# limix/CellRegMap

Hardware: AMD Instinct MI355X
Metric: variant-tests/sec (interaction test) (higher is better)
Workload: dtype f64

## Files before the change

cellregmap_amd/_lib.py:

```python
import ctypes
import os

import numpy as np

_HERE = os.path.dirname(os.path.abspath(__file__))
LIB_PATH = os.path.join(_HERE, "libcrm_hip.so")

c_double_p = ctypes.POINTER(ctypes.c_double)
c_int_p = ctypes.POINTER(ctypes.c_int)
c_long_p = ctypes.POINTER(ctypes.c_long)
vp = ctypes.c_void_p

SIGNATURES = {
    "crm_last_error": (ctypes.c_char_p, []),
    "crm_version": (ctypes.c_char_p, []),
    "crm_ctx_create": (ctypes.c_int, [ctypes.c_int, ctypes.POINTER(vp)]),
    "crm_ctx_destroy": (None, [vp]),
    "crm_ctx_synchronize": (ctypes.c_int, [vp]),
    "crm_ctx_trim": (ctypes.c_int, [vp]),
    "crm_background_create_qs": (ctypes.c_int, [vp, ctypes.c_long, ctypes.c_int, vp, vp, vp, vp,
                                                ctypes.POINTER(vp)]),
    "crm_background_create": (ctypes.c_int, [vp, ctypes.c_long, vp, ctypes.c_int, vp, ctypes.c_long,
                                             ctypes.c_int, vp, ctypes.c_double, ctypes.POINTER(vp)]),
    "crm_background_create_hadamard": (ctypes.c_int, [vp, ctypes.c_long, vp, ctypes.c_int, vp, ctypes.c_int, vp,
# ... 50 lines not shown
    "crm_set_progress_callback": (ctypes.c_int, [vp, vp, vp]),
    "crm_set_fast_rotation": (ctypes.c_int, [vp, ctypes.c_int]),
    "crm_kernel_timer_reset": (ctypes.c_int, [vp]),
    "crm_kernel_timer_read": (ctypes.c_int, [vp, c_double_p, c_long_p, c_double_p, c_double_p]),
    "crm_kernel_timer_stop": (ctypes.c_int, [vp]),
    "crm_test_set_form": (ctypes.c_int, [ctypes.c_char_p, ctypes.c_int, ctypes.c_int]),
    "crm_test_set_contraction": (ctypes.c_int, [vp, ctypes.c_int, ctypes.c_int]),
    "crm_test_set_shared_h": (ctypes.c_int, [vp, ctypes.c_int]),
    "crm_test_tail_launches": (ctypes.c_long, [vp]),
    "crm_test_spectrum_tail_launches": (ctypes.c_long, [vp]),
    "crm_test_dense_repeats": (ctypes.c_long, [vp]),
    "crm_test_donor_pair_blocks": (ctypes.c_long, [vp]),
    "crm_test_unrelated_donor_blocks": (ctypes.c_int, [vp, ctypes.POINTER(ctypes.c_long)]),
    "crm_test_gram_dma_launches": (ctypes.c_int, [vp, ctypes.POINTER(ctypes.c_long)]),
    "crm_test_fused_blocks": (ctypes.c_int, [vp, ctypes.POINTER(ctypes.c_long)]),
    "crm_test_rho0_position_blocks": (ctypes.c_int, [vp, ctypes.POINTER(ctypes.c_long)]),
    "crm_test_rotation_tail_launches": (ctypes.c_int, [vp, ctypes.POINTER(ctypes.c_long)]),
    "crm_test_tests_without_pair": (ctypes.c_long, [vp]),
    "crm_test_set_contraction_sync": (ctypes.c_int, [vp, ctypes.c_int]),
    "crm_test_sync_fallbacks": (ctypes.c_long, [vp]),
    "crm_test_overruns": (ctypes.c_long, []),
    "crm_test_live_device_bytes": (ctypes.c_long, []),
    "crm_test_set_kinship_route": (ctypes.c_int, [vp, ctypes.c_int]),
    "crm_test_check_context": (ctypes.c_int, [vp]),
    "crm_test_overrun_selftest": (ctypes.c_int, [vp]),
    "crm_test_null_fit_probe": (ctypes.c_int, [vp, ctypes.c_int, ctypes.c_double]),
    "crm_test_null_fit_probe_read": (ctypes.c_int, [vp, vp, ctypes.c_long]),
    "crm_test_contract": (ctypes.c_int, [vp, ctypes.c_long, ctypes.c_int, ctypes.c_int, vp, vp, vp,
                                         ctypes.c_int]),
    "crm_test_contract_kr": (ctypes.c_int, [vp, ctypes.c_long, ctypes.c_int, ctypes.c_int, ctypes.c_int,
# ... 52 lines not shown
```

cellregmap_amd/csrc/api_core.hip:

```cpp
#include <dlfcn.h>

#include <algorithm>
#include <atomic>
#include <cstdarg>
#include <mutex>

#include <map>

#include "crm_internal.h"
#include "eigh.h"

namespace crm {

static thread_local std::string g_error;

void set_error(const char* fmt, ...) {
    char buf[1024];
    va_list ap;
    va_start(ap, fmt);
    vsnprintf(buf, sizeof buf, fmt, ap);
    va_end(ap);
    g_error = buf;
}

// ... 258 lines not shown
    if (!c) return CRM_ERR_ARG;
    c->fast_T = on != 0;
    return CRM_OK;
    });
}

extern "C++" {
namespace crm {
namespace {
struct FormSlot { const char* name; int value; bool set; };
FormSlot g_forms[] = {{"gram_staged", 0, false}, {"kr_no_tail", 0, false}, {"nullfit_per_wave", 0, false}, {"kin_fold", 0, false},
                      {"eigh_one_stage", 0, false}, {"nullfit_exact", 0, false}, {"donor_pairs", 0, false},
                      {"pairs_without_kinship_term", 0, false}, {"flat_kappa_milli", 0, false}, {"chase_abort", 0, false}, {"nullfit_one_per_wave", 0, false},
                      {"kin_diag", 0, false}, {"donor_pairs_rotate", 0, false}, {"rho0_positions", 0, false},
                      {"rotation_tails", 0, false}, {"woodbury_ytY", 0, false},
                      {"wb_block_order", 0, false}, {"block_fused", 0, false}};
std::mutex g_forms_mu;
}
int form(const char* name, int otherwise) {
    std::lock_guard<std::mutex> lock(g_forms_mu);
    for (const FormSlot& f : g_forms)
        if (strcmp(f.name, name) == 0) return f.set ? f.value : otherwise;
    return otherwise;
}
}
}

int crm_test_set_form(const char* name, int value, int reset) {
    return crm::guarded("crm_test_set_form", [&]() -> int {
    if (!name) return CRM_ERR_ARG;
    std::lock_guard<std::mutex> lock(crm::g_forms_mu);
// ... 23 lines not shown
    return CRM_OK;
    });
}
int crm_test_unrelated_donor_blocks(const crm_ctx* ctx, long* blocks) {
    return crm::guarded("crm_test_unrelated_donor_blocks", [&]() -> int {
    if (!ctx || !blocks) return CRM_ERR_ARG;
    *blocks = ctx->unrelated_donor_blocks;
    return CRM_OK;
    });
}

int crm_test_fused_blocks(const crm_ctx* ctx, long* blocks) {
    return crm::guarded("crm_test_fused_blocks", [&]() -> int {
    if (!ctx || !blocks) return CRM_ERR_ARG;
    *blocks = ctx->fused_blocks;
    return CRM_OK;
    });
}

int crm_test_rho0_position_blocks(const crm_ctx* ctx, long* blocks) {
    return crm::guarded("crm_test_rho0_position_blocks", [&]() -> int {
    if (!ctx || !blocks) return CRM_ERR_ARG;
    *blocks = ctx->rho0_position_blocks;
    return CRM_OK;
    });
}
int crm_test_rotation_tail_launches(const crm_ctx* ctx, long* launches) {
    return crm::guarded("crm_test_rotation_tail_launches", [&]() -> int {
    if (!ctx || !launches) return CRM_ERR_ARG;
    *launches = ctx->rotation_tail_launches;
// ... 323 lines not shown
```

cellregmap_amd/csrc/assemble.hip:

```cpp
#include <type_traits>

#include "nullfit.h"

namespace crm {

namespace {

constexpr int CH = 64;
constexpr int SLD = 66;

typedef double v4d __attribute__((ext_vector_type(4)));

template <int NTL, int NG = 1>
__global__ __launch_bounds__(256) void gram_ext_kernel(AssembleArgs a, double* __restrict__ Gext, int KT) {
    constexpr int ROWS = 16 * NTL, NTILES = NTL * (NTL + 1) / 2, NLOC = (NTILES + NG - 1) / NG, MAXT = (NLOC + 3) / 4,
                  RPT = ROWS / 4;
    extern __shared__ double Ss[];
    __shared__ int tile_ij[NTILES];
    __shared__ const double* tail_ptr[ROWS];
    const int b = blockIdx.x;
    const NullFitOut fit = a.fit[b];
    const AssembleRho R = a.rho[fit.rho_index];
    const int r = R.r;
    const double ratio = fit.v0 / fit.v1;
// ... 809 lines not shown
            return CRM_ERR_INTERNAL;
        }
        Gext = a.wb_Gw;
    }
    const int P = a.c + 1;
    const size_t fin_small = sizeof(double) * ((size_t)P * P + 3 * P + a.k0);
    size_t fin_lds = fin_small + sizeof(double) * 2 * (size_t)a.k0 * P;
    const bool rows_global = fin_lds > 150 * 1024;
    if (rows_global) fin_lds = fin_small;
    if (a.k0 > CRM_MAX_K0 || a.c > CRM_MAX_COV_XWIDE || KT > CRM_MAX_GRAM_ROWS || (rows_global && !fin_rows)) {
        set_error("assemble: k0=%d, c=%d outside the supported range (k0 <= %d, c <= %d, k0 + c + 2 <= %d)", a.k0, a.c,
                  CRM_MAX_K0, CRM_MAX_COV_XWIDE, CRM_MAX_GRAM_ROWS);
        return CRM_ERR_UNSUPPORTED;
    }
    const int ts = (KT + 15) / 16;
    bool dma = ts <= 9 && a.ldA % 2 == 0 && (reinterpret_cast<uintptr_t>(a.A) & 15) == 0 && !form("gram_staged", 0);
    for (int i = 0; dma && i < CRM_MAX_RHO; i++) {
        const AssembleRho& R = a.rho[i];
        if (R.r <= 0 && !R.ty) continue;
        dma = R.ldW % 2 == 0 && R.ldT % 2 == 0 && ((reinterpret_cast<uintptr_t>(R.ty) | reinterpret_cast<uintptr_t>(R.tW) |
                                                    reinterpret_cast<uintptr_t>(R.T)) & 15) == 0;
    }
    if (a.wb_k1 > 0) dma = dma && a.wb_ldR % 2 == 0 && (reinterpret_cast<uintptr_t>(a.wb_R) & 15) == 0;
#define CRM_GRAM_DMA(KERNEL, LDS_DOUBLES, NTL)                                                                \
    do {                                                                                                      \
        const size_t lds = sizeof(double) * LDS_DOUBLES(NTL);                                                 \
        if (lds > 60 * 1024)                                                                                  \
            CRM_HIP(hipFuncSetAttribute(reinterpret_cast<const void*>(&KERNEL<NTL>),                          \
                                        hipFuncAttributeMaxDynamicSharedMemorySize, (int)lds));               \
        hipLaunchKernelGGL(KERNEL<NTL>, dim3(variants), dim3(256), lds, st, a, Gext, KT);                     \
    } while (0)
#define CRM_GRAM_DMA_WIDE(NTL) CRM_GRAM_DMA(gram_ext_dma_wide_kernel, gram_dma_wide_lds_doubles, NTL)
    if (dma) {
        if (ts <= 2) CRM_GRAM_DMA(gram_ext_dma_kernel, gram_dma_lds_doubles, 2);
        else if (ts <= 4) CRM_GRAM_DMA(gram_ext_dma_kernel, gram_dma_lds_doubles, 4);
        else if (ts == 5) CRM_GRAM_DMA_WIDE(5);
        else if (ts == 6) CRM_GRAM_DMA_WIDE(6);
        else if (ts == 7) CRM_GRAM_DMA_WIDE(7);
        else if (ts == 8) CRM_GRAM_DMA_WIDE(8);
        else CRM_GRAM_DMA_WIDE(9);
    }
#undef CRM_GRAM_DMA_WIDE
#undef CRM_GRAM_DMA
#define CRM_GRAM(NTL)                                                                                         \
    do {                                                                                                      \
        const size_t lds = sizeof(double) * 16 * NTL * SLD;                                                   \
        if (lds > 60 * 1024)                                                                                  \
            CRM_HIP(hipFuncSetAttribute(reinterpret_cast<const void*>(&gram_ext_kernel<NTL>),                 \
                                        hipFuncAttributeMaxDynamicSharedMemorySize, (int)lds));               \
        hipLaunchKernelGGL(gram_ext_kernel<NTL>, dim3(variants), dim3(256), lds, st, a, Gext, KT);            \
    } while (0)
#define CRM_GRAM_GROUPS(NTL, NG)                                                                              \
    do {                                                                                                      \
        const size_t lds = sizeof(double) * 16 * NTL * SLD;                                                   \
        CRM_HIP(hipFuncSetAttribute(reinterpret_cast<const void*>(&gram_ext_kernel<NTL, NG>),                 \
                                    hipFuncAttributeMaxDynamicSharedMemorySize, (int)lds));                   \
        hipLaunchKernelGGL((gram_ext_kernel<NTL, NG>), dim3(variants, NG), dim3(256), lds, st, a, Gext, KT);  \
    } while (0)
    if (dma) {
    } else if (ts <= 2) CRM_GRAM(2);
    else if (ts <= 4) CRM_GRAM(4);
    else if (ts <= 6) CRM_GRAM(6);
    else if (ts <= 7) CRM_GRAM(7);
    else if (ts <= 9) CRM_GRAM(9);
    else if (ts <= 12) CRM_GRAM_GROUPS(12, 2);
    else if (ts <= 15) CRM_GRAM_GROUPS(15, 4);
    else CRM_GRAM_GROUPS(18, 4);
#undef CRM_GRAM
#undef CRM_GRAM_GROUPS
    CRM_HIP(hipGetLastError());
    if (dma && dma_launches) ++*dma_launches;
    const bool yty = a.wb_k1 > 0 && form("woodbury_ytY", 1) != 0;
    if (a.wb_k1 > 0) {
        const size_t lds = yty ? sizeof(double) * a.wb_k1 * (size_t)((KT0 + a.wb_k1) | 1) : woodbury_lds_bytes(KT0, a.wb_k1);
        const void* fn = yty ? reinterpret_cast<const void*>(&woodbury_yty_kernel) : reinterpret_cast<const void*>(&woodbury_kernel);
        if (lds > 60 * 1024) CRM_HIP(hipFuncSetAttribute(fn, hipFuncAttributeMaxDynamicSharedMemorySize, (int)lds));
        if (yty) hipLaunchKernelGGL(woodbury_yty_kernel, dim3(variants), dim3(256), lds, st, a, a.wb_Gw, KT0, Gfin);
        else hipLaunchKernelGGL(woodbury_kernel, dim3(variants), dim3(256), lds, st, a, a.wb_Gw, KT0, Gfin);
        CRM_HIP(hipGetLastError());
    }
    if (fin_lds > 60 * 1024)
        CRM_HIP(hipFuncSetAttribute(reinterpret_cast<const void*>(&finalize_kernel),
                                    hipFuncAttributeMaxDynamicSharedMemorySize, (int)fin_lds));
    hipLaunchKernelGGL(finalize_kernel, dim3(variants), dim3(128), fin_lds, st, a, Gfin, KT0, rows_global ? fin_rows : nullptr,
                       yty ? 1 : 0);
    CRM_HIP(hipGetLastError());
// ... 5 lines not shown
```

cellregmap_amd/csrc/crm_internal.h:

```cpp
#pragma once
#include <map>
#include <mutex>
#include <thread>
#include <type_traits>
#include <utility>

#include "crm_common.h"

namespace crm {

constexpr int CRM_DEFAULT_BLOCK = 1024;
constexpr int CRM_MAX_AUTO_BLOCK = 4096;
constexpr int CRM_MAX_RHO = 16;
constexpr int CRM_MAX_COV = 8;
constexpr int CRM_MAX_COV_WIDE = 62;
constexpr int CRM_MAX_COV_XWIDE = 128;
constexpr int CRM_MAX_K0 = 256;
constexpr int CRM_MAX_GRAM_ROWS = 288;
constexpr int DT_SUMS_LD = 136;
constexpr int BLOCK_SLACK_MAX = 4096;

struct DevBuf {
    void* ptr = nullptr;
    size_t bytes = 0;
// ... 57 lines not shown
    bool probe_on = false;
    int probe_mode = 0;
    double probe_x = 0.0;
    std::vector<double> probe_out;
    bool nullfit_exact = false;
    crm::GemmTune tune;
    crm::DevBuf sync_counters;
    unsigned* sync_timeouts_host = nullptr;
    long sync_fallbacks = 0;
    long dense_repeats = 0;
    long tail_launches = 0;
    long spectrum_tail_launches = 0;
    long donor_pair_blocks = 0;
    long rotation_tail_launches = 0;
    long rho0_position_blocks = 0;
    long fused_blocks = 0;
    long unrelated_donor_blocks = 0;
    long gram_dma_launches = 0;
    long tests_without_pair = 0;
    struct ReplayBlock {
        long col0 = 0;
        int nb = 0;
        bool collapsed = false;
        std::vector<char> fit;
        crm::DevBuf T;
    };
    int replay_mode = 0;
    size_t replay_cursor = 0;
    std::vector<ReplayBlock*> replay_blocks;
    void replay_clear() {
// ... 46 lines not shown
```

cellregmap_amd/csrc/nullfit.h:

```cpp
#pragma once
#include "crm_internal.h"

namespace crm {

struct NullFitRho {
    const double* T;
    const double* ty;
    const double* tW;
    const double* S0;
    long ldT, ldW;
    int r;
    int pad_;
};

struct NullFitTrial {
    double lml, delta, scale;
    int use_g, nfev;
    double margin;
    double noise;
    double curv;
};

struct NullFitOut {
    int rho_index;
// ... 153 lines not shown
    const double* Z1; long ldZ1;
    const double* Z2; long ldZ2;
    const double* Z3; long ldZ3;
    const double* WW; const double* Wy; double yy;
    const double* gg; const double* gy; const double* gW; long ld_gW;
    const double* coef; long ld_coef;
    double* Q;
    double* F;
    int wb_k1;
    const double* wb_R; long wb_ldR;
    const double* wb_E1X; long wb_ldE1X;
    const double* wb_E1yW; long wb_ldE1yW;
    const double* wb_E1g; long wb_ldE1g;
    const double* wb_EE;
    double* wb_Gw;
};

int launch_assemble(hipStream_t st, const AssembleArgs& a, int variants, double* Gext, double* fin_rows = nullptr,
                    long* dma_launches = nullptr);
size_t assemble_rows_scratch_doubles(int variants, int k0, int c);
size_t woodbury_lds_bytes(int KT, int k1);

int launch_eig_davies(hipStream_t st, const double* F, const double* Q, int count, int k,
                      double* lambda, double* pvalue, int* ifault, double* liu, bool do_eig, double* scratch = nullptr,
                      int* trace = nullptr);
size_t eig_scratch_doubles(int count, int k);

int launch_tail_pvalue(hipStream_t st, const double* Q, const double* lambda, int count, int k, double* pvalue,
                       double* logp, int* status);

}
```

cellregmap_amd/csrc/scan_pairs.hip:

```cpp
#include "scan_pass.h"

namespace crm {

SubRange ScanPass::sub_range(const Block& B, int b0) const {
    SubRange R;
    R.b0 = b0;
    R.nb = B.nb - b0;
    R.done = B.done + b0;
    if (ng > 1) {
        long pairs = 0;
        int take = 0;
        for (; b0 + take < B.nb; take++) {
            unsigned seen = 0;
            for (int gi = 0; gi < ng; gi++) {
                const NullFitOut& f = h_fit[(size_t)gi * P.BLK + b0 + take];
                if (!no_kinship_term(f)) seen |= 1u << f.rho_index;
            }
            const int here = __builtin_popcount(seen);
            if (take > 0 && pairs + here > P.pair_cap) break;
            pairs += here;
        }
        R.nb = take;
    }
    return R;
// ... 182 lines not shown
        const long s0 = sps * per, s1 = std::min(stages_all, s0 + per);
        if (s1 <= s0) break;
        GemmProblem& e = kp[groups + slices++];
        e.X = D.G + s0 * GEMM_BK * D.ldg; e.ldx = D.ldg;
        e.E = d_Ep + s0 * GEMM_BK * g0->ld_ep; e.lde = g0->ld_ep; e.k0 = k0;
        e.Y = bg->H.as<double>() + s0 * GEMM_BK * bg->ldh; e.ldy = bg->ldh;
        e.C = ctx->ws_AH.as<double>() + (size_t)sps * e1_slab; e.ldc = ld_ah;
        e.M = ncol * k0; e.N = k1; e.cells = (s1 - s0) * GEMM_BK;
        chunk_max = std::max(chunk_max, e.cells);
    }
    kp.resize((size_t)groups + std::max(slices, 1));
    return with_records(SLOT_KIN, kp, [&](GemmProblem* d_kp) -> int {
        double* AH = ctx->ws_AH.as<double>();
        if (probed.donor_pairs) {
            CRM_TRY(launch_gemm_tn(ctx, d_kp, (int)groups, ncol, npair, maxlen, false, 0, 1, 0));
            if (probed.wb_rotate)
                CRM_TRY(launch_donor_pairs_rotate(st, ctx->ws_Pd.as<double>(), P.pd_slab, P.ldPd, (int)groups, ncol, k0,
                                                  bg->wb_U.as<double>(), (long)bg->wb_k2pad * 128, 128, bg->wb_k2pad,
                                                  ctx->ws_A.as<double>(), P.ldAw, AH, P.pd_slab, P.donor_pair_splits));
            else
                CRM_TRY(launch_donor_pairs_expand(st, ctx->ws_Pd.as<double>(), P.pd_slab, P.ldPd, (int)groups, ncol, k0, k1, S, ld_ah,
                                                  AH, P.pd_slab, P.donor_pair_splits));
            CRM_TRY(launch_reduce_splits(st, AH, (long)ncol * P.ldPd, P.donor_pair_splits, P.pd_slab));
            CRM_TRY(launch_pair_rows_sym(st, AH, P.ldPd, ncol, k0, S, ld_ah));
            ctx->donor_pair_blocks++;
        } else {
            if (k2 == 1) CRM_TRY(launch_gemm_tn(ctx, d_kp, (int)groups, ncol, k0, maxlen, false, 0, 1, 0));
            else CRM_TRY(launch_kr_transposed(ctx, d_kp, (int)groups, ncol * k0, k2, maxlen, k0));
            if (P.e1_pairs) {
                const long p_slab = (long)(std::max<long>(P.BLK, P.pair_cap) + 128) * P.ldP;
                CRM_TRY(launch_gemm_tn(ctx, d_kp + groups, 1, ncol, probed.e1_sym ? npair : k1 * k0, np, false, 0, P.fold_split6, p_slab));
// ... 56 lines not shown
        return CRM_OK;
    });
}

int ScanPass::direct_AH(const Block& B, const SubRange& R, const Pairs& Q, AGroups& A) {
    GemmProblem p{};
    p.X = B.Gt + R.b0; p.ldx = B.ldt; p.E = d_Ep; p.lde = g0->ld_ep; p.k0 = k0; p.Y = bg->H.as<double>(); p.ldy = bg->ldh;
    p.C = ctx->ws_AH.as<double>(); p.ldc = P.ld_ah; p.M = R.nb * k0; p.N = (int)bg->cols;
    CRM_TRY(upload(SLOT_ONE, &p, 1));
    CRM_TRY(launch_kr_transposed(ctx, d_probs + SLOT_ONE, 1, p.M, p.N, np, k0));
    A.kr_flops += 2.0 * (double)n * (double)bg->cols * (double)k0 * (double)R.nb;
    return gather_pairs(ctx->ws_AH.as<double>(), bg->ldh, Q);
}

int ScanPass::woodbury_S(const SubRange& R, const Pairs& Q) {
    const long groups = bg->kin_groups;
    const int ncol = P.wb_block ? R.nb : Q.npairs;
    std::vector<GemmProblem> kp((size_t)groups);
    GemmProblem p{};
    p.X = ctx->ws_S.as<double>() + (size_t)bg->kin_k1 * P.ld_ah; p.ldx = P.ld_ah;
    p.C = ctx->ws_A.as<double>(); p.ldc = P.ldAw; p.M = ncol * k0;
    woodbury_records(bg, p, (long)bg->kin_k2 * P.ld_ah, kp.data());
    return with_records(SLOT_KIN, kp, [&](GemmProblem* d_kp) {
        return launch_gemm_tn(ctx, d_kp, (int)groups, ncol * k0, bg->kin_k2, bg->wb_k2pad, false, 0, 1, 0);
    });
}

int ScanPass::form_A(const Block& B, const SubRange& R, const Pairs& Q) {
    bool via_H = P.kin();
    if (P.fastT && ng > 1 && !P.kin()) {
        double direct = 0.0, via = (double)R.nb * (double)bg->cols * (double)n;
        for (int i = 0; i < nrho; i++) {
            direct += (double)Q.cnt[i] * bg->r[i] * (double)n;
            via += (double)Q.cnt[i] * bg->r[i] * (double)bg->ldh;
        }
        via_H = ctx->tune.shared_h < 0 ? via < 0.9 * direct : ctx->tune.shared_h > 0;
    }
    const bool direct = !P.collapsed() && !via_H;
    if (direct)
        for (int i = 0; i < nrho; i++)
            if (Q.cnt[i] > 0) CRM_TRY(crm_background_require_q0(bg, i));
    AGroups A;
    bool tail_of[CRM_MAX_RHO] = {false};
// ... 91 lines not shown
```

cellregmap_amd/csrc/scan_pass.h:

```cpp
#pragma once
#include <algorithm>
#include <vector>

#include "nullfit.h"
#include "objects.h"

namespace crm {

int ctx_cus(const crm_ctx* ctx);

constexpr double COLLINEAR_TAU = 1e-2;

constexpr double STOP_SHIFT_C = 2.5e-13;
constexpr double FLAT_KAPPA = 1.0;
constexpr double RHO_KAPPA = 1.0;
constexpr int FLAT_REC = 10;

struct ScanOut {
    double *pv, *rho1, *e2, *g2, *eps2, *Q, *lml, *delta, *scale, *lambda, *F;
    int* ifault = nullptr;
    double* liu = nullptr;
    int* flags = nullptr;
    double* bound_Q = nullptr;
    double* bound_p = nullptr;
// ... 94 lines not shown
    double *dZ1 = nullptr, *dZ2 = nullptr, *dZ3 = nullptr;
    long z1_sz = 0, z2_sz = 0, z3_sz = 0;
    double *d_gg, *d_gy, *d_gW, *d_Q, *d_pv, *d_lam, *d_liu, *d_part, *d_coef, *d_thr, *d_tp, *d_tlp;
    int *d_pos, *d_ord, *d_if, *d_drop, *d_near, *d_posw, *d_tst;
    NullFitTrial* d_trial;
    NullFitOut* d_fit;
    unsigned* d_queue;
    double *wb_yW = nullptr, *wb_E1yW = nullptr, *wb_g = nullptr, *wb_Gw = nullptr, *wb_tmp = nullptr;
    std::vector<NullFitOut> h_fit = std::vector<NullFitOut>((size_t)P.BLK * ng);
    std::vector<int> h_pos = std::vector<int>((size_t)P.BLK * ng), h_ord = std::vector<int>(P.pair_cap);
    std::vector<GemmProblem> probs = std::vector<GemmProblem>(CRM_MAX_RHO + 4);
    std::vector<int> pair_of = std::vector<int>((size_t)nrho * P.BLK), h_near = std::vector<int>(P.BLK);
    bool rho0_pos[CRM_MAX_RHO] = {false};
    std::vector<GemmProblem> rot_tails;
    std::vector<GemmProblem> phi_recs;

    ScanPass(const std::vector<crm_gene*>& genes_, crm_panel* panel_, long first_, long count_, const int* idx_E_,
             const int* idx_G_, const std::vector<ScanOut>& outs_, bool allow_collapse, std::vector<long>* near_out_)
        : genes(genes_), panel(panel_), first(first_), count(count_), idx_E(idx_E_), idx_G(idx_G_), outs(outs_),
          near_out(near_out_), ng((int)genes_.size()), g0(genes_[0]), bg(g0->bg), ctx(bg->ctx), st(ctx->stream), n(bg->n),
          np(bg->n_pad), ldq(bg->ldq), slab((long)(1 + g0->c) * bg->ldq), nrho(bg->nrho), c(g0->c), k0(g0->k0),
          P(plan_scan(genes_, panel_, idx_G_, allow_collapse, count_)) {}

    int upload(int slot, const GemmProblem* p, size_t k) {
        CRM_HIP(hipMemcpyAsync(d_probs + slot, p, sizeof(GemmProblem) * k, hipMemcpyHostToDevice, st));
        return CRM_OK;
    }
    template <class F>
    int with_records(int slot, const std::vector<GemmProblem>& kp, F&& launches) {
        CRM_TRY(upload(slot, kp.data(), kp.size()));
// ... 44 lines not shown
    SubRange sub_range(const Block& B, int b0) const;
    int select_pairs(const Block& B, const SubRange& R, Pairs& Q);
    int direct_splits(const Pairs& Q, AGroups& A, bool* tail_of);
    void a_records(const Pairs& Q, bool via_H, const bool* tail_of, AGroups& A);
    int donor_columns(const Block& B, const SubRange& R, const Pairs& Q, DonorCols& D);
    int gather_pairs(const double* src, long rows, const Pairs& Q);
    int folded_S(const Block& B, const SubRange& R, const Pairs& Q);
    int unfolded_AH(const Block& B, const SubRange& R, const Pairs& Q);
    int direct_AH(const Block& B, const SubRange& R, const Pairs& Q, AGroups& A);
    int woodbury_S(const SubRange& R, const Pairs& Q);
    int form_A(const Block& B, const SubRange& R, const Pairs& Q);
    int side_contractions(const Block& B, const SubRange& R);
    int z1_products(const Block& B, const SubRange& R);
    int flat_probes(const Block& B, const SubRange& R, int gi, const AssembleArgs& aa, double* slow_ws, std::vector<char>& flat,
                    std::vector<double>& probe_rec);
    int gene_results(const Block& B, const SubRange& R, int gi);
};

}
```

cellregmap_amd/csrc/scan_prepare.hip:

```cpp
#include "scan_pass.h"

namespace crm {

long donor_run_records(const crm_background* bg, const GemmProblem& p, long c_step, GemmProblem* out) {
    long maxlen = GEMM_BK;
    for (long d = 0; d < bg->kin_groups; d++) {
        const long r0 = bg->kin_row0[d];
        GemmProblem q = p;
        q.X = p.X + r0 * p.ldx;
        if (p.E) q.E = p.E + r0 * p.lde;
        q.Y = p.Y + r0 * p.ldy; q.C = p.C + d * c_step; q.cells = bg->kin_len[d];
        maxlen = std::max(maxlen, bg->kin_len[d]);
        out[d] = q;
    }
    return maxlen;
}

void woodbury_records(const crm_background* bg, const GemmProblem& p, long x_step, GemmProblem* out) {
    for (long d = 0; d < bg->kin_groups; d++) {
        GemmProblem q = p;
        q.X = p.X + d * x_step; q.Y = bg->wb_U.as<double>() + (size_t)d * bg->wb_k2pad * 128; q.ldy = 128;
        q.C = p.C + d * bg->kin_k2; q.N = bg->kin_k2; q.cells = bg->wb_k2pad;
        out[d] = q;
    }
// ... 1 lines not shown

int same_columns(hipStream_t st, int* d_flag, int k, std::initializer_list<SameColumns> pairs, bool& same) {
    int h_flag = 0;
    CRM_HIP(hipMemsetAsync(d_flag, 0, sizeof(int), st));
    for (const SameColumns& q : pairs) CRM_TRY(launch_same_columns(st, q.A, q.lda, q.B, q.ldb, q.rows, k, d_flag));
    CRM_HIP(hipMemcpyAsync(&h_flag, d_flag, sizeof(int), hipMemcpyDeviceToHost, st));
    CRM_HIP(hipStreamSynchronize(st));
    same = h_flag == 0;
    return CRM_OK;
}

int ScanPass::workspaces() {
    const int BLK = P.BLK, max_pairs = P.pair_cap;
    const long ldb = P.ldb;
    CRM_TRY(ctx->ws_T.ensure(sizeof(double) * (size_t)nrho * BLK * P.ldT));
    CRM_TRY(ctx->ws_A.ensure(sizeof(double) * (size_t)(P.wb() ? std::max(max_pairs, BLK) : max_pairs) * k0 * P.ldAw));
    CRM_TRY(ctx->ws_Anone.ensure(sizeof(double) * (size_t)P.ldAw));
    CRM_HIP(hipMemsetAsync(ctx->ws_Anone.ptr, 0, sizeof(double) * (size_t)P.ldAw, st));
    bool copies = false, fused = false;
    for (long done = 0; done < count; done += BLK)
        (fused_block(first + done, (int)std::min<long>(BLK, count - done)) ? fused : copies) = true;
    if (copies) CRM_TRY(ctx->ws_Gb.ensure(sizeof(double) * (size_t)np * ldb));
    if (fused && P.kin() && (ng > 1 || P.wb_block))
        CRM_TRY(ctx->ws_Gkt.ensure(sizeof(double) * (size_t)bg->kin_rows * ldb));
    CRM_TRY(ctx->ws_Gs.ensure(sizeof(double) * (size_t)np * P.ldp));
    CRM_TRY(ctx->ws_G2.ensure(sizeof(double) * (size_t)np * ldb));
    if (idx_G)
        CRM_TRY(ctx->ws_Gt.ensure(sizeof(double) * (size_t)np * ldb));
    z1_sz = (long)BLK * P.ldZ1, z2_sz = (long)BLK * P.ldZ2, z3_sz = (long)BLK * P.ldZ3;
    const long z1_all = z1_sz * P.ks1 * ng;
    CRM_TRY(ctx->ws_Z.ensure(sizeof(double) * (size_t)(z1_all + z2_sz * P.ks2 + z3_sz * P.ks3)));
// ... 285 lines not shown
```

cellregmap_amd/csrc/scan_results.hip:

```cpp
#include "scan_pass.h"

namespace crm {

__global__ void flat_probe_fit_kernel(const crm::NullFitOut* __restrict__ fit, int count, double sign,
                                      crm::NullFitOut* __restrict__ out) {
    const int b = blockIdx.x * blockDim.x + threadIdx.x;
    if (b >= count) return;
    crm::NullFitOut f = fit[b];
    const double tiny = 2.220446049250313e-16;
    const double d = fmin(fmax(f.delta, tiny), 1.0 - tiny);
    const double x = log(d) - log1p(-d);
    const double tol = 1e-6 * fabs(x) + 1e-6;
    const double dp = fmin(fmax(1.0 / (1.0 + exp(-(x + sign * tol))), tiny), 1.0 - tiny);
    f.delta = dp;
    f.v0 = 1.0 - dp;
    f.v1 = dp;
    f.scale = -1.0;
    out[b] = f;
}

int ScanPass::flat_probes(const Block& B, const SubRange& R, int gi, const AssembleArgs& aa, double* slow_ws, std::vector<char>& flat,
                std::vector<double>& probe_rec) {
    const ScanOut& o = outs[gi];
    const int nb = R.nb;
// ... 35 lines not shown
    for (int b = 0; b < nb; b++) {
        const NullFitOut& fo = fit[b];
        const double* rec = &probe_rec[(size_t)b * FLAT_REC];
        const double gain = fo.curv / std::fabs(fo.lml);
        double shift = (gain > 0.0 && gain == gain) ? std::min(1.0, STOP_SHIFT_C / gain) : 1.0;
        if (!(rec[0] > flat_kappa)) shift = 1.0;
        const double bq = rec[1] * shift, bp = rec[2] * shift;
        if (o.bound_Q) o.bound_Q[R.done + b] = bq;
        if (o.bound_p) o.bound_p[R.done + b] = bp;
        if (!(bp <= 1e-5)) flat[b] |= 1;
        if (!(bq <= 1e-6)) flat[b] |= 2;
    }
    return CRM_OK;
}

int ScanPass::gene_results(const Block& B, const SubRange& R, int gi) {
    crm_gene* g = genes[gi];
    const ScanOut& o = outs[gi];
    const int nb = R.nb, BLK = P.BLK, b0 = R.b0;
    const long done = R.done;
    AssembleArgs aa{};
    for (int i = 0; i < nrho; i++) {
        AssembleRho& Rr = aa.rho[i];
        Rr.ty = g->rot.as<double>() + (long)i * slab;
        Rr.tW = Rr.ty + ldq; Rr.ldW = ldq;
        Rr.S0 = bg->S0[i].as<double>();
        Rr.T = ctx->ws_T.as<double>() + ((size_t)i * BLK + b0) * P.ldT; Rr.ldT = P.ldT;
        Rr.r = bg->r[i];
    }
    aa.fit = d_fit + (size_t)gi * BLK + b0; aa.sorted_pos = d_pos + (size_t)gi * BLK;
    aa.A = ctx->ws_A.as<double>(); aa.ldA = P.ldA; aa.k0 = k0; aa.c = c; aa.n = n; aa.A_none = ctx->ws_Anone.as<double>();
    aa.Z1 = dZ1 + (size_t)gi * z1_sz * P.ks1; aa.ldZ1 = P.ldZ1; aa.Z2 = dZ2; aa.ldZ2 = P.ldZ2; aa.Z3 = dZ3; aa.ldZ3 = P.ldZ3;
    aa.WW = g->WW.as<double>(); aa.Wy = g->Wy.as<double>(); aa.yy = g->yy;
    aa.gg = d_gg + b0; aa.gy = d_gy + b0 + (size_t)gi * BLK; aa.gW = d_gW + (size_t)b0 * P.ld_gW; aa.ld_gW = P.ld_gW;
    aa.coef = P.collapsed() ? nullptr : d_coef + b0; aa.ld_coef = P.ldb; aa.Q = d_Q; aa.F = ctx->ws_F.as<double>();
// ... 1 lines not shown
    if (P.wb()) {
        for (int i = 0; i < nrho; i++) {
            AssembleRho& Rr = aa.rho[i];
            Rr.ty = wb_yW + (size_t)gi * (1 + c) * P.ldwb;
            Rr.tW = Rr.ty + P.ldwb; Rr.ldW = P.ldwb;
            Rr.S0 = bg->wb_S0[i].as<double>();
            Rr.T = wb_g + (size_t)b0 * P.ldwb; Rr.ldT = P.ldwb;
            Rr.r = (int)bg->wb_P;
        }
        aa.sorted_pos = (ng == 1 ? d_pos : d_posw) + (size_t)gi * BLK; aa.A = ctx->ws_A.as<double>(); aa.ldA = P.ldAw;
        aa.wb_k1 = bg->kin_k1; aa.wb_R = bg->wb_R.as<double>(); aa.wb_ldR = P.ldwb;
        aa.wb_E1X = ctx->ws_S.as<double>(); aa.wb_ldE1X = P.ld_ah;
        aa.wb_E1yW = wb_E1yW + (size_t)gi * bg->kin_k1 * 128; aa.wb_ldE1yW = 128;
        aa.wb_E1g = ctx->ws_TH.as<double>() + b0; aa.wb_ldE1g = P.ldb; aa.wb_EE = bg->wb_EE.as<double>(); aa.wb_Gw = wb_Gw;
    }
    double* slow_ws = P.slow_forms ? ctx->ws_xwide.as<double>() : nullptr;
    CRM_TRY(launch_assemble(st, aa, nb, ctx->ws_Gext.as<double>(), slow_ws, &ctx->gram_dma_launches));
    CRM_TRY(launch_eig_davies(st, ctx->ws_F.as<double>(), d_Q, nb, k0, d_lam, d_pv, d_if, d_liu, true, slow_ws));
    if (o.exact) {
        CRM_TRY(launch_tail_pvalue(st, d_Q, d_lam, nb, k0, d_tp, d_tlp, d_tst));
        if (o.logp) CRM_HIP(hipMemcpyAsync(o.logp + done, d_tlp, sizeof(double) * nb, hipMemcpyDeviceToHost, st));
        if (o.status) CRM_HIP(hipMemcpyAsync(o.status + done, d_tst, sizeof(int) * nb, hipMemcpyDeviceToHost, st));
    }
    if (o.pv) CRM_HIP(hipMemcpyAsync(o.pv + done, o.exact ? d_tp : d_pv, sizeof(double) * nb, hipMemcpyDeviceToHost, st));
    if (o.Q) CRM_HIP(hipMemcpyAsync(o.Q + done, d_Q, sizeof(double) * nb, hipMemcpyDeviceToHost, st));
    if (o.lambda) CRM_HIP(hipMemcpyAsync(o.lambda + done * k0, d_lam, sizeof(double) * nb * k0, hipMemcpyDeviceToHost, st));
    if (o.F) CRM_HIP(hipMemcpyAsync(o.F + done * k0 * k0, ctx->ws_F.ptr, sizeof(double) * nb * k0 * k0, hipMemcpyDeviceToHost, st));
    if (o.ifault) CRM_HIP(hipMemcpyAsync(o.ifault + done, d_if, sizeof(int) * nb, hipMemcpyDeviceToHost, st));
    if (o.liu) CRM_HIP(hipMemcpyAsync(o.liu + done, d_liu, sizeof(double) * nb, hipMemcpyDeviceToHost, st));
    std::vector<char> flat;
// ... 37 lines not shown
```

Measured before the change: 77190.

## Fuse unrelated-donor pair rotation with Woodbury Gram assembly in one kernel

Adds a kernel that, per variant, rotates the donor-pair products through U into an LDS image and immediately accumulates the extended Gram matrix with f64 MFMA. It uses async global-to-LDS DMA and double-buffers the per-donor chunks. This removes the separate rotate kernel, the write and re-read of the A workspace, and the Gram launch inside assembly. The allocation of ws_A is deferred when fusion may apply. It only runs under narrow shape and alignment conditions, and in exchange it carries high LDS and register use and limits occupancy.

Measured after the change: 78750 (median of 6 runs). 1.02x the previous value.

```diff
diff --git a/cellregmap_amd/_lib.py b/cellregmap_amd/_lib.py
--- a/cellregmap_amd/_lib.py
+++ b/cellregmap_amd/_lib.py
@@ -88,6 +88,7 @@
     "crm_test_unrelated_donor_blocks": (ctypes.c_int, [vp, ctypes.POINTER(ctypes.c_long)]),
     "crm_test_gram_dma_launches": (ctypes.c_int, [vp, ctypes.POINTER(ctypes.c_long)]),
     "crm_test_fused_blocks": (ctypes.c_int, [vp, ctypes.POINTER(ctypes.c_long)]),
+    "crm_test_wb_gram_fused_blocks": (ctypes.c_int, [vp, ctypes.POINTER(ctypes.c_long)]),
     "crm_test_rho0_position_blocks": (ctypes.c_int, [vp, ctypes.POINTER(ctypes.c_long)]),
     "crm_test_rotation_tail_launches": (ctypes.c_int, [vp, ctypes.POINTER(ctypes.c_long)]),
     "crm_test_tests_without_pair": (ctypes.c_long, [vp]),
diff --git a/cellregmap_amd/csrc/api_core.hip b/cellregmap_amd/csrc/api_core.hip
--- a/cellregmap_amd/csrc/api_core.hip
+++ b/cellregmap_amd/csrc/api_core.hip
@@ -296,7 +296,7 @@
                       {"pairs_without_kinship_term", 0, false}, {"flat_kappa_milli", 0, false}, {"chase_abort", 0, false}, {"nullfit_one_per_wave", 0, false},
                       {"kin_diag", 0, false}, {"donor_pairs_rotate", 0, false}, {"rho0_positions", 0, false},
                       {"rotation_tails", 0, false}, {"woodbury_ytY", 0, false},
-                      {"wb_block_order", 0, false}, {"block_fused", 0, false}};
+                      {"wb_block_order", 0, false}, {"block_fused", 0, false}, {"wb_gram_fused", 0, false}};
 std::mutex g_forms_mu;
 }
 int form(const char* name, int otherwise) {
@@ -350,6 +350,14 @@
     return crm::guarded("crm_test_fused_blocks", [&]() -> int {
     if (!ctx || !blocks) return CRM_ERR_ARG;
     *blocks = ctx->fused_blocks;
+    return CRM_OK;
+    });
+}
+
+int crm_test_wb_gram_fused_blocks(const crm_ctx* ctx, long* blocks) {
+    return crm::guarded("crm_test_wb_gram_fused_blocks", [&]() -> int {
+    if (!ctx || !blocks) return CRM_ERR_ARG;
+    *blocks = ctx->wb_gram_fused_blocks;
     return CRM_OK;
     });
 }
diff --git a/cellregmap_amd/csrc/assemble.hip b/cellregmap_amd/csrc/assemble.hip
--- a/cellregmap_amd/csrc/assemble.hip
+++ b/cellregmap_amd/csrc/assemble.hip
@@ -847,6 +847,7 @@
         return CRM_ERR_UNSUPPORTED;
     }
     const int ts = (KT + 15) / 16;
+    const bool gram_done = a.wb_k1 > 0 && a.wb_gram_done != 0;
     bool dma = ts <= 9 && a.ldA % 2 == 0 && (reinterpret_cast<uintptr_t>(a.A) & 15) == 0 && !form("gram_staged", 0);
     for (int i = 0; dma && i < CRM_MAX_RHO; i++) {
         const AssembleRho& R = a.rho[i];
@@ -864,7 +865,8 @@
         hipLaunchKernelGGL(KERNEL<NTL>, dim3(variants), dim3(256), lds, st, a, Gext, KT);                     \
     } while (0)
 #define CRM_GRAM_DMA_WIDE(NTL) CRM_GRAM_DMA(gram_ext_dma_wide_kernel, gram_dma_wide_lds_doubles, NTL)
-    if (dma) {
+    if (gram_done) {
+    } else if (dma) {
         if (ts <= 2) CRM_GRAM_DMA(gram_ext_dma_kernel, gram_dma_lds_doubles, 2);
         else if (ts <= 4) CRM_GRAM_DMA(gram_ext_dma_kernel, gram_dma_lds_doubles, 4);
         else if (ts == 5) CRM_GRAM_DMA_WIDE(5);
@@ -890,7 +892,7 @@
                                     hipFuncAttributeMaxDynamicSharedMemorySize, (int)lds));                   \
         hipLaunchKernelGGL((gram_ext_kernel<NTL, NG>), dim3(variants, NG), dim3(256), lds, st, a, Gext, KT);  \
     } while (0)
-    if (dma) {
+    if (dma || gram_done) {
     } else if (ts <= 2) CRM_GRAM(2);
     else if (ts <= 4) CRM_GRAM(4);
     else if (ts <= 6) CRM_GRAM(6);
@@ -902,7 +904,7 @@
 #undef CRM_GRAM
 #undef CRM_GRAM_GROUPS
     CRM_HIP(hipGetLastError());
-    if (dma && dma_launches) ++*dma_launches;
+    if ((dma || gram_done) && dma_launches) ++*dma_launches;
     const bool yty = a.wb_k1 > 0 && form("woodbury_ytY", 1) != 0;
     if (a.wb_k1 > 0) {
         const size_t lds = yty ? sizeof(double) * a.wb_k1 * (size_t)((KT0 + a.wb_k1) | 1) : woodbury_lds_bytes(KT0, a.wb_k1);
diff --git a/cellregmap_amd/csrc/crm_internal.h b/cellregmap_amd/csrc/crm_internal.h
--- a/cellregmap_amd/csrc/crm_internal.h
+++ b/cellregmap_amd/csrc/crm_internal.h
@@ -95,6 +95,7 @@
     long donor_pair_blocks = 0;
     long rotation_tail_launches = 0;
     long rho0_position_blocks = 0;
+    long wb_gram_fused_blocks = 0;
     long fused_blocks = 0;
     long unrelated_donor_blocks = 0;
     long gram_dma_launches = 0;
diff --git a/cellregmap_amd/csrc/nullfit.h b/cellregmap_amd/csrc/nullfit.h
--- a/cellregmap_amd/csrc/nullfit.h
+++ b/cellregmap_amd/csrc/nullfit.h
@@ -191,6 +191,7 @@
     const double* wb_E1g; long wb_ldE1g;
     const double* wb_EE;
     double* wb_Gw;
+    int wb_gram_done;
 };
 
 int launch_assemble(hipStream_t st, const AssembleArgs& a, int variants, double* Gext, double* fin_rows = nullptr,
@@ -198,6 +199,17 @@
 size_t assemble_rows_scratch_doubles(int variants, int k0, int c);
 size_t woodbury_lds_bytes(int KT, int k1);
 
+struct WbFusedArgs {
+    const double* P; long p_slab, ldp;
+    const double* U; long u_slab, ldu;
+    double* Psum; long psum_slab;
+    int donors, splits, k2pad;
+};
+struct WbFusedLayout { int RS, UW, urows, rows_o, nP, nU, nO, off_P, off_U, off_S0, off_d, off_rp, total; };
+WbFusedLayout wb_gram_fused_layout(int k0, int KT, long ldp);
+bool wb_gram_fused_serves(const AssembleArgs& a, const WbFusedArgs& f, int nrho);
+int launch_wb_gram_fused(hipStream_t st, const AssembleArgs& a, const WbFusedArgs& f, int nrho, int variants);
+
 int launch_eig_davies(hipStream_t st, const double* F, const double* Q, int count, int k,
                       double* lambda, double* pvalue, int* ifault, double* liu, bool do_eig, double* scratch = nullptr,
                       int* trace = nullptr);
diff --git a/cellregmap_amd/csrc/scan_pairs.hip b/cellregmap_amd/csrc/scan_pairs.hip
--- a/cellregmap_amd/csrc/scan_pairs.hip
+++ b/cellregmap_amd/csrc/scan_pairs.hip
@@ -220,7 +220,19 @@
         double* AH = ctx->ws_AH.as<double>();
         if (probed.donor_pairs) {
             CRM_TRY(launch_gemm_tn(ctx, d_kp, (int)groups, ncol, npair, maxlen, false, 0, 1, 0));
-            if (probed.wb_rotate)
+            if (probed.wb_rotate && may_fuse_gram() && R.b0 == 0 && R.nb == B.nb) {
+                const AssembleArgs aa = assemble_args(R, 0);
+                const WbFusedArgs fa{ctx->ws_Pd.as<double>(), P.pd_slab, P.ldPd, bg->wb_U.as<double>(), (long)bg->wb_k2pad * 128, 128,
+                                     AH, P.pd_slab, (int)groups, P.donor_pair_splits, bg->wb_k2pad};
+                if (wb_gram_fused_serves(aa, fa, nrho)) {
+                    CRM_TRY(launch_wb_gram_fused(st, aa, fa, nrho, ncol));
+                    gram_fused = true;
+                    ctx->wb_gram_fused_blocks++;
+                }
+            }
+            if (!gram_fused && P.wb()) CRM_TRY(ctx->ws_A.ensure(ws_A_bytes()));
+            if (gram_fused) {
+            } else if (probed.wb_rotate)
                 CRM_TRY(launch_donor_pairs_rotate(st, ctx->ws_Pd.as<double>(), P.pd_slab, P.ldPd, (int)groups, ncol, k0,
                                                   bg->wb_U.as<double>(), (long)bg->wb_k2pad * 128, 128, bg->wb_k2pad,
                                                   ctx->ws_A.as<double>(), P.ldAw, AH, P.pd_slab, P.donor_pair_splits));
@@ -307,6 +319,7 @@
 }
 
 int ScanPass::woodbury_S(const SubRange& R, const Pairs& Q) {
+    CRM_TRY(ctx->ws_A.ensure(ws_A_bytes()));
     const long groups = bg->kin_groups;
     const int ncol = P.wb_block ? R.nb : Q.npairs;
     std::vector<GemmProblem> kp((size_t)groups);
@@ -320,6 +333,7 @@
 }
 
 int ScanPass::form_A(const Block& B, const SubRange& R, const Pairs& Q) {
+    gram_fused = false;
     bool via_H = P.kin();
     if (P.fastT && ng > 1 && !P.kin()) {
         double direct = 0.0, via = (double)R.nb * (double)bg->cols * (double)n;
diff --git a/cellregmap_amd/csrc/scan_pass.h b/cellregmap_amd/csrc/scan_pass.h
--- a/cellregmap_amd/csrc/scan_pass.h
+++ b/cellregmap_amd/csrc/scan_pass.h
@@ -132,6 +132,7 @@
     bool rho0_pos[CRM_MAX_RHO] = {false};
     std::vector<GemmProblem> rot_tails;
     std::vector<GemmProblem> phi_recs;
+    bool gram_fused = false;
 
     ScanPass(const std::vector<crm_gene*>& genes_, crm_panel* panel_, long first_, long count_, const int* idx_E_,
              const int* idx_G_, const std::vector<ScanOut>& outs_, bool allow_collapse, std::vector<long>* near_out_)
@@ -206,6 +207,15 @@
     int z1_products(const Block& B, const SubRange& R);
     int flat_probes(const Block& B, const SubRange& R, int gi, const AssembleArgs& aa, double* slow_ws, std::vector<char>& flat,
                     std::vector<double>& probe_rec);
+    AssembleArgs assemble_args(const SubRange& R, int gi) const;
+    size_t ws_A_bytes() const {
+        return sizeof(double) * (size_t)(P.wb() ? std::max(P.pair_cap, P.BLK) : P.pair_cap) * k0 * P.ldAw;
+    }
+    bool may_fuse_gram() const {
+        const int ts = (2 * k0 + c + 2 + 15) / 16;
+        return P.wb_rotate && ng == 1 && P.wb_block && !outs[0].flags && ctx->replay_mode == 0 && k0 % 2 == 0 && ts >= 5 && ts <= 8 &&
+               form("wb_gram_fused", 1) != 0 && form("gram_staged", 0) == 0;
+    }
     int gene_results(const Block& B, const SubRange& R, int gi);
 };
 
diff --git a/cellregmap_amd/csrc/scan_prepare.hip b/cellregmap_amd/csrc/scan_prepare.hip
--- a/cellregmap_amd/csrc/scan_prepare.hip
+++ b/cellregmap_amd/csrc/scan_prepare.hip
@@ -39,7 +39,7 @@
     const int BLK = P.BLK, max_pairs = P.pair_cap;
     const long ldb = P.ldb;
     CRM_TRY(ctx->ws_T.ensure(sizeof(double) * (size_t)nrho * BLK * P.ldT));
-    CRM_TRY(ctx->ws_A.ensure(sizeof(double) * (size_t)(P.wb() ? std::max(max_pairs, BLK) : max_pairs) * k0 * P.ldAw));
+    if (!may_fuse_gram()) CRM_TRY(ctx->ws_A.ensure(ws_A_bytes()));
     CRM_TRY(ctx->ws_Anone.ensure(sizeof(double) * (size_t)P.ldAw));
     CRM_HIP(hipMemsetAsync(ctx->ws_Anone.ptr, 0, sizeof(double) * (size_t)P.ldAw, st));
     bool copies = false, fused = false;
diff --git a/cellregmap_amd/csrc/scan_results.hip b/cellregmap_amd/csrc/scan_results.hip
--- a/cellregmap_amd/csrc/scan_results.hip
+++ b/cellregmap_amd/csrc/scan_results.hip
@@ -73,11 +73,9 @@
     return CRM_OK;
 }
 
-int ScanPass::gene_results(const Block& B, const SubRange& R, int gi) {
+AssembleArgs ScanPass::assemble_args(const SubRange& R, int gi) const {
     crm_gene* g = genes[gi];
-    const ScanOut& o = outs[gi];
-    const int nb = R.nb, BLK = P.BLK, b0 = R.b0;
-    const long done = R.done;
+    const int BLK = P.BLK, b0 = R.b0;
     AssembleArgs aa{};
     for (int i = 0; i < nrho; i++) {
         AssembleRho& Rr = aa.rho[i];
@@ -109,6 +107,15 @@
         aa.wb_E1yW = wb_E1yW + (size_t)gi * bg->kin_k1 * 128; aa.wb_ldE1yW = 128;
         aa.wb_E1g = ctx->ws_TH.as<double>() + b0; aa.wb_ldE1g = P.ldb; aa.wb_EE = bg->wb_EE.as<double>(); aa.wb_Gw = wb_Gw;
     }
+    return aa;
+}
+
+int ScanPass::gene_results(const Block& B, const SubRange& R, int gi) {
+    const ScanOut& o = outs[gi];
+    const int nb = R.nb, BLK = P.BLK, b0 = R.b0;
+    const long done = R.done;
+    AssembleArgs aa = assemble_args(R, gi);
+    aa.wb_gram_done = gram_fused ? 1 : 0;
     double* slow_ws = P.slow_forms ? ctx->ws_xwide.as<double>() : nullptr;
     CRM_TRY(launch_assemble(st, aa, nb, ctx->ws_Gext.as<double>(), slow_ws, &ctx->gram_dma_launches));
     CRM_TRY(launch_eig_davies(st, ctx->ws_F.as<double>(), d_Q, nb, k0, d_lam, d_pv, d_if, d_liu, true, slow_ws));
diff --git a/cellregmap_amd/csrc/wb_gram_fused.hip b/cellregmap_amd/csrc/wb_gram_fused.hip
--- /dev/null
+++ b/cellregmap_amd/csrc/wb_gram_fused.hip
@@ -0,0 +1,328 @@
+#include <type_traits>
+
+#include "nullfit.h"
+
+namespace crm {
+
+namespace {
+
+typedef double v4d __attribute__((ext_vector_type(4)));
+typedef const double __attribute__((address_space(1))) * fused_gptr_t;
+typedef __attribute__((address_space(3))) void* fused_lptr_t;
+
+__device__ __forceinline__ void fused_dma16(const double* src, double* lds_wave_uniform) {
+    __builtin_amdgcn_global_load_lds((fused_gptr_t)src, (fused_lptr_t)lds_wave_uniform, 16, 0, 0);
+}
+
+__device__ __forceinline__ void dma_barrier() { asm volatile("s_waitcnt vmcnt(0) lgkmcnt(0)\n\ts_barrier" ::: "memory"); }
+
+constexpr int WF_MAXQ_P = 10, WF_MAXQ_O = 9, WF_PSUM = 6;
+constexpr int WF_UW = 56;
+
+}
+
+WbFusedLayout wb_gram_fused_layout(int k0, int KT, long ldp) {
+    WbFusedLayout L;
+    const int KS = (k0 + 3) / 4;
+    L.urows = 4 * KS;
+    L.UW = WF_UW;
+    L.RS = (k0 + 4) | 2;
+    L.nP = (int)(ldp / 128);
+    L.nU = (L.urows * (L.UW / 2) + 63) / 64;
+    L.rows_o = KT - k0;
+    L.nO = (L.rows_o * (L.RS / 2) + 63) / 64;
+    L.off_P = k0 * L.RS + L.nO * 128;
+    L.off_U = L.off_P + L.nP * 128;
+    L.off_S0 = L.off_U + L.nU * 128;
+    L.off_d = L.off_S0 + 128;
+    L.off_rp = L.off_d + 64;
+    L.total = L.off_rp + ((L.rows_o + 1) & ~1);
+    return L;
+}
+
+namespace {
+
+template <int NTL>
+__global__ __launch_bounds__(256, NTL <= 7 ? 2 : 1) void wb_gram_fused_kernel(AssembleArgs a, WbFusedArgs f, WbFusedLayout L, int KT) {
+    constexpr int NTILES = NTL * (NTL + 1) / 2, MAXT = (NTILES + 3) / 4;
+    extern __shared__ __align__(16) double smem[];
+    double* const img = smem;
+    double* const Pl = smem + L.off_P;
+    double* const Ul = smem + L.off_U;
+    double* const S0l = smem + L.off_S0;
+    double* const dS = smem + L.off_d;
+    const double** const rowp = reinterpret_cast<const double**>(smem + L.off_rp);
+    const int b = blockIdx.x;
+    const NullFitOut fit = a.fit[b];
+    const AssembleRho R = a.rho[fit.rho_index];
+    const double ratio = fit.v0 / fit.v1;
+    const bool has_A = a.sorted_pos[b] >= 0;
+    const int tid = threadIdx.x;
+    const int lane = tid & 63, wave = __builtin_amdgcn_readfirstlane(tid >> 6);
+    const int l15 = lane & 15, lq = lane >> 4;
+    const int k0 = a.k0, c = a.c, RS = L.RS;
+    constexpr int UW = WF_UW;
+    const int npair = k0 * (k0 + 1) / 2, KS = (k0 + 3) / 4, JT = (k0 + 15) / 16;
+    const int D = f.donors, Ptot = D * k0;
+    const double* __restrict__ zeros = a.A_none;
+
+    for (int e = tid; e < k0 * RS; e += 256) img[e] = 0.0;
+    for (int t = tid; t < L.rows_o; t += 256) {
+        const double* p;
+        if (t < c) p = R.tW + (long)t * R.ldW;
+        else if (t == c) p = R.T + (long)b * R.ldT;
+        else if (t == c + 1) p = R.ty;
+        else p = a.wb_R + (long)(t - c - 2) * a.wb_ldR;
+        rowp[t] = p;
+    }
+    const int nPU = L.nP + L.nU + 1;
+    int poff[WF_MAXQ_P], ocode[WF_MAXQ_O];
+#pragma unroll
+    for (int q = 0; q < WF_MAXQ_P; q++) {
+        const int I = wave + 4 * q;
+        if (I < L.nP) poff[q] = 128 * I + 2 * lane;
+        else if (I < L.nP + L.nU) {
+            const int u = 64 * (I - L.nP) + lane, k = u / (UW / 2), cu = u - k * (UW / 2);
+            poff[q] = k < L.urows ? k * (int)f.ldu + 2 * cu : 0;
+        } else poff[q] = 2 * lane;
+    }
+#pragma unroll
+    for (int q = 0; q < WF_MAXQ_O; q++) {
+        const int u = 64 * (wave + 4 * q) + lane, t = u / (RS / 2), cu = u - t * (RS / 2);
+        ocode[q] = t < L.rows_o ? (t << 8) | (2 * cu) : -1;
+    }
+    auto chunk = [&](int d, int& start, int& end, int& c0, int& lim) __attribute__((always_inline)) {
+        start = (k0 * d) & ~3;
+        end = d + 1 < D ? (k0 * (d + 1)) & ~3 : (Ptot + 3) & ~3;
+        c0 = 2 - (k0 * d - start);
+        lim = end < Ptot ? end : Ptot;
+    };
+    auto issue_pus = [&](int d) __attribute__((always_inline)) {
+        int start, end, c0, lim;
+        chunk(d, start, end, c0, lim);
+        const double* __restrict__ Pd = f.P + (size_t)d * f.p_slab + (long)b * f.ldp;
+        const double* __restrict__ Ud = f.U + (size_t)d * f.u_slab;
+        const double* __restrict__ S0 = R.S0 + (start - c0);
+#pragma unroll
+        for (int q = 0; q < WF_MAXQ_P; q++) {
+            const int I = wave + 4 * q;
+            if (I < L.nP) fused_dma16(Pd + poff[q], Pl + 128 * I);
+            else if (I < L.nP + L.nU) fused_dma16(Ud + poff[q], Ul + 128 * (I - L.nP));
+            else if (I < nPU) {
+                const int col = poff[q];
+                fused_dma16(col >= c0 && start - c0 + col < lim ? S0 + col : zeros, S0l);
+            }
+        }
+    };
+    auto issue_others = [&](int d) __attribute__((always_inline)) {
+        int start, end, c0, lim;
+        chunk(d, start, end, c0, lim);
+        const int shift = start - c0;
+#pragma unroll
+        for (int q = 0; q < WF_MAXQ_O; q++) {
+            const int I = wave + 4 * q;
+            if (I < L.nO) {
+                const int code = ocode[q], col = code & 255;
+                const bool in = code >= 0 && col >= c0 && shift + col < lim;
+                const double* src = zeros;
+                if (in) src = rowp[code >> 8] + (shift + col);
+                fused_dma16(src, img + k0 * RS + 128 * I);
+            }
+        }
+    };
+    const int iw = 16 * wave + l15;
+    int pidx[16];
+#pragma unroll
+    for (int ks = 0; ks < 16; ks++) {
+        const int k = 4 * ks + lq, lo = k < iw ? k : iw, hi = k < iw ? iw : k;
+        pidx[ks] = k < k0 && iw < k0 ? lo * k0 - lo * (lo - 1) / 2 + (hi - lo) : 0;
+    }
+    const int first = (wave + b) & 3;
+    const int ntw = (NTILES - first + 3) / 4;
+    int t_i[MAXT], t_j[MAXT], t_ij[MAXT];
+#pragma unroll
+    for (int t = 0; t < MAXT; t++) {
+        int ti = 0, rem = first + 4 * t < NTILES ? first + 4 * t : 0;
+        while (rem >= NTL - ti) { rem -= NTL - ti; ti++; }
+        t_ij[t] = ti | ((ti + rem) << 8);
+        const int ri = 16 * ti + l15, rj = 16 * (ti + rem) + l15;
+        t_i[t] = (ri < KT ? ri : 0) * RS + lq;
+        t_j[t] = (rj < KT ? rj : 0) * RS + lq;
+    }
+    v4d acc[MAXT];
+#pragma unroll
+    for (int t = 0; t < MAXT; t++) acc[t] = (v4d){0.0, 0.0, 0.0, 0.0};
+    double psum[WF_PSUM];
+#pragma unroll
+    for (int q = 0; q < WF_PSUM; q++) psum[q] = 0.0;
+    const int per = (D + f.splits - 1) / f.splits;
+    int split = 0;
+
+    auto gram = [&](int col0, int nks, auto nt_tag) __attribute__((always_inline)) {
+        constexpr int NT = decltype(nt_tag)::value;
+        const double* __restrict__ S = img + col0;
+        const double* __restrict__ Dw = dS + col0 + lq;
+        double fa[NT], fr[NT];
+        double dk = Dw[0];
+#pragma unroll
+        for (int t = 0; t < NT; t++) {
+            fa[t] = S[t_i[t]];
+            fr[t] = S[t_j[t]];
+        }
+        for (int ks = 0; ks < nks; ks++) {
+            const bool more = ks + 1 < nks;
+            const int nx = more ? 4 * (ks + 1) : 4 * ks;
+            const double dn = Dw[nx];
+#pragma unroll
+            for (int t = 0; t < NT; t++) {
+                acc[t] = __builtin_amdgcn_mfma_f64_16x16x4f64(fa[t], fr[t] * dk, acc[t], 0, 0, 0);
+                fa[t] = S[t_i[t] + nx];
+                fr[t] = S[t_j[t] + nx];
+            }
+            dk = dn;
+        }
+    };
+
+    __syncthreads();
+    issue_pus(0);
+    issue_others(0);
+    dma_barrier();
+    for (int d = 0; d < D; d++) {
+        int start, end, c0, lim;
+        chunk(d, start, end, c0, lim);
+        if (tid < RS) {
+#pragma clang fp contract(off)
+            const double s = ratio * S0l[tid];
+            dS[tid] = s / (1.0 + s);
+        }
+#pragma unroll
+        for (int q = 0; q < WF_PSUM; q++)
+            if (tid + 256 * q < npair) psum[q] += Pl[tid + 256 * q];
+        if (d + 1 == D || d + 1 == (split + 1) * per) {
+            double* __restrict__ out = f.Psum + (size_t)split * f.psum_slab + (long)b * f.ldp;
+#pragma unroll
+            for (int q = 0; q < WF_PSUM; q++)
+                if (tid + 256 * q < npair) { out[tid + 256 * q] = psum[q]; psum[q] = 0.0; }
+            split++;
+        }
+        if (has_A && wave < JT) {
+            unsigned uo = (unsigned)(lq * UW + l15);
+            asm volatile("" : "+v"(uo));
+            const double* __restrict__ ub = Ul + uo;
+            const int jcut = end - k0 * d;
+#pragma unroll
+            for (int th = 0; th < 4; th += 2) {
+                if (th < JT) {
+                    v4d cr[2];
+#pragma unroll
+                    for (int t = 0; t < 2; t++) cr[t] = (v4d){0.0, 0.0, 0.0, 0.0};
+                    double af[3], bf[3][2];
+                    auto frag = [&](int ks, int slot) __attribute__((always_inline)) {
+                        af[slot] = Pl[pidx[ks]];
+#pragma unroll
+                        for (int t = 0; t < 2; t++)
+                            if (th + t < JT) bf[slot][t] = ub[4 * ks * UW + 16 * (th + t)];
+                    };
+                    frag(0, 0);
+                    if (1 < KS) frag(1, 1);
+#pragma unroll
+                    for (int ks = 0; ks < 16; ks++) {
+                        if (ks < KS) {
+                            if (ks + 2 < KS) frag(ks + 2, (ks + 2) % 3);
+#pragma unroll
+                            for (int t = 0; t < 2; t++)
+                                if (th + t < JT)
+                                    cr[t] = __builtin_amdgcn_mfma_f64_16x16x4f64(af[ks % 3], bf[ks % 3][t], cr[t], 0, 0, 0);
+                            __builtin_amdgcn_sched_barrier(0);
+                        }
+                    }
+#pragma unroll
+                    for (int reg = 0; reg < 4; reg++) {
+                        const int r = 16 * wave + lq + 4 * reg;
+                        if (r < k0) {
+#pragma unroll
+                            for (int t = 0; t < 2; t++) {
+                                const int j = 16 * (th + t) + l15;
+                                if (th + t < JT && j < k0) img[r * RS + (j < jcut ? j + 2 : j - jcut)] = cr[t][reg];
+                            }
+                        }
+                    }
+                }
+            }
+        }
+        dma_barrier();
+        if (d + 1 < D) issue_pus(d + 1);
+        const int nks = (end - start) / 4;
+        if (ntw == MAXT) gram(c0, nks, std::integral_constant<int, MAXT>{});
+        else gram(c0, nks, std::integral_constant<int, MAXT - 1>{});
+        dma_barrier();
+        if (d + 1 < D) issue_others(d + 1);
+    }
+    for (; split < f.splits; split++) {
+        double* __restrict__ out = f.Psum + (size_t)split * f.psum_slab + (long)b * f.ldp;
+        for (int e = tid; e < npair; e += 256) out[e] = 0.0;
+    }
+    double* __restrict__ out = a.wb_Gw + (long)b * KT * KT;
+#pragma unroll
+    for (int t = 0; t < MAXT; t++) {
+        if (t >= ntw) continue;
+        const int ri = (t_ij[t] & 255) * 16, cj = (t_ij[t] >> 8) * 16;
+#pragma unroll
+        for (int reg = 0; reg < 4; reg++) {
+            const int row = ri + lq + 4 * reg, col = cj + l15;
+            if (row < KT && col < KT) {
+                out[(long)row * KT + col] = acc[t][reg];
+                if (ri != cj) out[(long)col * KT + row] = acc[t][reg];
+            }
+        }
+    }
+}
+
+bool aligned16(const void* p) { return (reinterpret_cast<uintptr_t>(p) & 15) == 0; }
+
+}
+
+bool wb_gram_fused_serves(const AssembleArgs& a, const WbFusedArgs& f, int nrho) {
+    const int k0 = a.k0, KT = k0 + a.c + 2 + a.wb_k1, ts = (KT + 15) / 16;
+    if (form("wb_gram_fused", 1) == 0 || form("gram_staged", 0) != 0) return false;
+    if (a.wb_k1 <= 0 || k0 % 2 != 0 || !donor_pairs_rotate_serves(k0) || ts < 5 || ts > 8 || f.donors < 1 || f.splits < 1) return false;
+    if (f.ldp % 128 != 0 || f.ldp < k0 * (k0 + 1) / 2 || f.p_slab % 2 != 0 || f.u_slab % 2 != 0 || f.ldu % 2 != 0 || f.ldu < 4 * ((k0 + 3) / 4) ||
+        f.k2pad < 4 * ((k0 + 3) / 4) || !aligned16(f.P) || !aligned16(f.U) || !aligned16(a.A_none) || !a.wb_Gw)
+        return false;
+    if (a.wb_ldR % 2 != 0 || !aligned16(a.wb_R)) return false;
+    for (int i = 0; i < nrho; i++) {
+        const AssembleRho& R = a.rho[i];
+        if (R.r != f.donors * k0 || R.ldW % 2 != 0 || R.ldT % 2 != 0 || !aligned16(R.ty) || !aligned16(R.tW) || !aligned16(R.T) ||
+            !aligned16(R.S0))
+            return false;
+    }
+    const WbFusedLayout L = wb_gram_fused_layout(k0, KT, f.ldp);
+    return L.nP + L.nU + 1 <= 4 * WF_MAXQ_P && L.nO <= 4 * WF_MAXQ_O && L.RS <= 64 && k0 * (k0 + 1) / 2 <= 256 * WF_PSUM &&
+           sizeof(double) * (size_t)L.total <= 160 * 1024;
+}
+
+int launch_wb_gram_fused(hipStream_t st, const AssembleArgs& a, const WbFusedArgs& f, int nrho, int variants) {
+    if (variants <= 0) return CRM_OK;
+    if (!wb_gram_fused_serves(a, f, nrho)) {
+        set_error("fused unrelated-donor Gram: k0=%d, c=%d outside the supported range", a.k0, a.c);
+        return CRM_ERR_INTERNAL;
+    }
+    const int KT = a.k0 + a.c + 2 + a.wb_k1, ts = (KT + 15) / 16;
+    const WbFusedLayout L = wb_gram_fused_layout(a.k0, KT, f.ldp);
+    const size_t lds = sizeof(double) * (size_t)L.total;
+#define CRM_WB_FUSED(NTL)                                                                                             \
+    do {                                                                                                              \
+        CRM_HIP(hipFuncSetAttribute(reinterpret_cast<const void*>(&wb_gram_fused_kernel<NTL>),                        \
+                                    hipFuncAttributeMaxDynamicSharedMemorySize, (int)lds));                           \
+        hipLaunchKernelGGL(wb_gram_fused_kernel<NTL>, dim3(variants), dim3(256), lds, st, a, f, L, KT);               \
+    } while (0)
+    if (ts == 5) CRM_WB_FUSED(5);
+    else if (ts == 6) CRM_WB_FUSED(6);
+    else if (ts == 7) CRM_WB_FUSED(7);
+    else CRM_WB_FUSED(8);
+#undef CRM_WB_FUSED
+    CRM_HIP(hipGetLastError());
+    return CRM_OK;
+}
+
+}
```
